# TencentARC/TVTS

Hardware: AMD Instinct MI355X
Metric: video-text pairs/sec/node, TVTSv2 pretrain step (higher is better)
Workload: dtype bf16; 1 GPU; TVTSv2 ViT-B/16 8-frame 224^2, mask 0.5, 32-token captions x4, full pretrain step (fwd+losses+bwd+HF-AdamW); pairs_per_gpu=192, global_batch=192, parallelism=dp1, hip_graph=False

## Files before the change

tvts_amd/csrc/attention.hip:

```cpp
#include "common.h"
#include <stdlib.h>

enum { MODE_FULL = 0, MODE_SPACE = 1, MODE_TIME = 2, MODE_CLS = 3 };
#ifndef TVTS_DH
#define TVTS_DH 64
#endif
#define DH TVTS_DH
#if TVTS_DH == 64
#define NS_DH dh64
#define ABI(name) tvts_attn_##name
#define VSTRIDE 160
#else
#define NS_DH dh80
#define ABI(name) tvts_attn80_##name
#define VSTRIDE 192
#endif
namespace NS_DH {
constexpr int DT = DH / 16;
constexpr int KS = (DH + 31) / 32;
constexpr int NCH = DH / 8;

struct AttnGeom {
    int B, heads, S, T, n;
    int causal;
// ... 1636 lines not shown
template <int MT, bool TR, int RS_ = 0>
__global__ __launch_bounds__(256) void attn_fwd_time_fused_kernel(AttnGeom g, const bf16* __restrict__ qkv,
                                                                  bf16* __restrict__ out, int ldo, float* __restrict__ lse2,
                                                                  float* __restrict__ cls_part) {
    extern __shared__ __attribute__((aligned(16))) char smem[];
    constexpr int RA = MT * 16, RS = RS_ ? RS_ : RA, TB = RS * VSTRIDE, NU = (MT + 1) / 2;
    constexpr int WB = TB + (DH + 2 + 2) * 4 + 1024;
    constexpr int PT = (RS * NCH + 63) / 64;
    const int lane = threadIdx.x & 63, wave = threadIdx.x >> 6;
    char* Vs = smem + wave * WB;
    char* opatch = Vs + TB + (DH + 4) * 4;
    const int chunks = (g.n + TIME_CHUNK - 1) / TIME_CHUNK;
    Grp r;
    r.h = blockIdx.x % g.heads;
    const int c = (blockIdx.x / g.heads) % chunks;
    r.b = blockIdx.x / (g.heads * chunks); r.nq = g.T; r.nk = g.T + 1;
    const int p_end = (c + 1) * TIME_CHUNK < g.n ? (c + 1) * TIME_CHUNK : g.n;
    const int gq = lane >> 4, li = lane & 15;
    const int hcol = r.h * DH;
    const int m = g.T + 1;
    float Mr = -1e30f, Lr = 0.f;
    f32x4 Or[DT];
#pragma unroll
    for (int dt = 0; dt < DT; ++dt) Or[dt] = (f32x4){0, 0, 0, 0};
    Q8Out q8o;
    q8o.init(g);

    bf16x8 qf[MT][KS], kf[MT][KS], vst[PT];
    auto issue = [&](int p) {
        r.sub = p;
#pragma unroll
        for (int t = 0; t < MT; ++t) {
            const int j = t * 16 + li;
            const bf16* rowp = qkv + (size_t)k_row<MODE_TIME>(g, r, j < m ? j : m - 1) * g.ld + hcol;
            ld_frags(rowp, gq, qf[t]);
            ld_frags(rowp + g.W, gq, kf[t]);
        }
#pragma unroll
        for (int i = 0; i < PT; ++i) {
            const int cc = lane + 64 * i, row = cc / NCH, ch = cc % NCH;
            vst[i] = row < m ? ldg8(qkv + (size_t)k_row<MODE_TIME>(g, r, row) * g.ld + 2 * g.W + hcol + ch * 8) : zero8();
        }
    };
    int p = c * TIME_CHUNK + wave;
    if (p < p_end) issue(p);
    for (; p < p_end; p += 4) {
#pragma unroll
        for (int i = 0; i < PT; ++i) {
            const int cc = lane + 64 * i, row = cc / NCH, ch = cc % NCH;
            if (row < RS) *(bf16x8*)(Vs + row * VSTRIDE + ch * 16) = vst[i];
        }
        bf16x8 qc[MT][KS], kc[MT][KS];
#pragma unroll
        for (int t = 0; t < MT; ++t)
#pragma unroll
            for (int ks = 0; ks < KS; ++ks) { qc[t][ks] = qf[t][ks]; kc[t][ks] = kf[t][ks]; }
        const bool first = p == 0;
        if (p + 4 < p_end) issue(p + 4);
        r.sub = p;
#pragma unroll
        for (int qt = 0; qt < MT; ++qt) {
            const int qj = qt * 16 + li;
            f32x4 st[2 * NU];
            float mx = -INFINITY;
#pragma unroll
            for (int t = 0; t < 2 * NU; ++t) {
                st[t] = (f32x4){-INFINITY, -INFINITY, -INFINITY, -INFINITY};
                if (t < MT) {
                    f32x4 sc = {0, 0, 0, 0};
#pragma unroll
                    for (int ks = 0; ks < KS; ++ks) sc = __builtin_amdgcn_mfma_f32_16x16x32_bf16(kc[t][ks], qc[qt][ks], sc, 0, 0, 0);
#pragma unroll
                    for (int e = 0; e < 4; ++e) {
                        const int key = t * 16 + gq * 4 + e;
                        const bool ok = key < m && !(key == 0 && qj == 0 && !first);
                        const float v = ok ? sc[e] * g.scale2 : -INFINITY;
                        st[t][e] = v;
                        mx = fmaxf(mx, v);
                    }
                }
            }
            mx = group_max(mx);
            float rs = 0.f;
#pragma unroll
            for (int t = 0; t < 2 * NU; ++t)
#pragma unroll
                for (int e = 0; e < 4; ++e) {
                    const float pp = __builtin_amdgcn_exp2f(st[t][e] - mx);
                    st[t][e] = pp;
                    rs += pp;
                }
            const float l = group_sum(rs);
            f32x4 o[DT];
#pragma unroll
            for (int dt = 0; dt < DT; ++dt) o[dt] = (f32x4){0, 0, 0, 0};
#pragma unroll
            for (int u = 0; u < NU; ++u) {
                bf16x8 pf;
#pragma unroll
                for (int j = 0; j < 8; ++j) pf[j] = (bf16)st[2 * u + (j >> 2)][j & 3];
#pragma unroll
                for (int dt = 0; dt < DT; ++dt)
                    o[dt] = __builtin_amdgcn_mfma_f32_16x16x32_bf16(frag_T_lim<TR>(Vs, u, dt, lane, RA, RS), pf, o[dt], 0, 0, 0);
            }
            {
                const float inv = 1.0f / l;
                f32x4 on[DT];
#pragma unroll
                for (int dt = 0; dt < DT; ++dt) on[dt] = o[dt] * inv;
                store_tile_rows(opatch, on, lane, [&](int rr) -> bf16* {
                    const int j = qt * 16 + rr;
                    return (j >= 1 && j < m) ? out + (size_t)k_row<MODE_TIME>(g, r, j) * ldo + hcol : nullptr; }, &q8o);
            }
            if (qj >= 1 && qj < m && gq == 0) lse2[(size_t)k_row<MODE_TIME>(g, r, qj) * g.heads + r.h] = mx + log2f(l);
            if (qt == 0) {
                const float Mn = fmaxf(Mr, mx);
                const float a = __builtin_amdgcn_exp2f(Mr - Mn), b = __builtin_amdgcn_exp2f(mx - Mn);
                Lr = Lr * a + l * b;
#pragma unroll
                for (int dt = 0; dt < DT; ++dt) Or[dt] = Or[dt] * a + o[dt] * b;
                Mr = Mn;
            }
        }
    }
    q8o.finish(g, lane);
    float* cst = (float*)(smem + wave * WB + TB);
    if (li == 0) {
        if (gq == 0) { cst[0] = Mr; cst[1] = Lr; }
#pragma unroll
        for (int dt = 0; dt < DT; ++dt)
#pragma unroll
            for (int e = 0; e < 4; ++e) cst[2 + dt * 16 + gq * 4 + e] = Or[dt][e];
    }
    __syncthreads();
    if (threadIdx.x < DH) {
        const int d = threadIdx.x;
        float M = -1e30f;
#pragma unroll
        for (int w = 0; w < 4; ++w) M = fmaxf(M, *(const float*)(smem + w * WB + TB));
        float L = 0.f, O = 0.f;
#pragma unroll
        for (int w = 0; w < 4; ++w) {
            const float* cw = (const float*)(smem + w * WB + TB);
            const float sc = __builtin_amdgcn_exp2f(cw[0] - M);
            L += cw[1] * sc;
            O += cw[2 + d] * sc;
        }
        float* cp = cls_part + ((size_t)(r.b * g.heads + r.h) * chunks + c) * (DH + 2);
        if (d == 0) { cp[0] = M; cp[1] = L; }
        cp[2 + d] = O;
    }
}

template <int MT, bool TR>
__global__ __launch_bounds__(256) void attn_fwd_seq_fused_kernel(AttnGeom g, const bf16* __restrict__ qkv,
                                                                 bf16* __restrict__ out, int ldo, float* __restrict__ lse2) {
    extern __shared__ __attribute__((aligned(16))) char smem[];
    constexpr int RA = MT * 16, TB = RA * VSTRIDE, NU = (MT + 1) / 2;
    constexpr int WB = TB + 1024;
    constexpr int PT = (RA * NCH + 63) / 64;
    const int lane = threadIdx.x & 63, wave = threadIdx.x >> 6;
    char* Vs = smem + wave * WB;
    char* opatch = Vs + TB;
    const int gq = lane >> 4, li = lane & 15;
    const int m = g.S, groups = g.B * g.heads, stride = gridDim.x * 4;
    const bool causal = g.causal != 0;

    bf16x8 qf[MT][KS], kf[MT][KS], vst[PT];
    auto issue = [&](int gid) {
        const bf16* base = qkv + (size_t)(gid / g.heads) * g.S * g.ld + (gid % g.heads) * DH;
#pragma unroll
        for (int t = 0; t < MT; ++t) {
            const int j = t * 16 + li;
            const bf16* rowp = base + (size_t)(j < m ? j : m - 1) * g.ld;
            ld_frags(rowp, gq, qf[t]);
            ld_frags(rowp + g.W, gq, kf[t]);
        }
#pragma unroll
        for (int i = 0; i < PT; ++i) {
            const int cc = lane + 64 * i, row = cc / NCH, ch = cc % NCH;
            vst[i] = row < m ? ldg8(base + (size_t)row * g.ld + 2 * g.W + ch * 8) : zero8();
        }
    };
    int gid = blockIdx.x * 4 + wave;
    if (gid < groups) issue(gid);
    for (; gid < groups; gid += stride) {
#pragma unroll
        for (int i = 0; i < PT; ++i) {
            const int cc = lane + 64 * i, row = cc / NCH, ch = cc % NCH;
            if (row < RA) *(bf16x8*)(Vs + row * VSTRIDE + ch * 16) = vst[i];
        }
        bf16x8 qc[MT][KS], kc[MT][KS];
#pragma unroll
        for (int t = 0; t < MT; ++t)
#pragma unroll
            for (int ks = 0; ks < KS; ++ks) { qc[t][ks] = qf[t][ks]; kc[t][ks] = kf[t][ks]; }
        if (gid + stride < groups) issue(gid + stride);
        const int h = gid % g.heads;
        const size_t row0 = (size_t)(gid / g.heads) * g.S;
        const int hcol = h * DH;
#pragma unroll
        for (int qt = 0; qt < MT; ++qt) {
            const int qj = qt * 16 + li;
            f32x4 st[2 * NU];
            float mx = -INFINITY;
#pragma unroll
            for (int t = 0; t < 2 * NU; ++t) {
                st[t] = (f32x4){-INFINITY, -INFINITY, -INFINITY, -INFINITY};
                if (t < MT) {
                    f32x4 sc = {0, 0, 0, 0};
#pragma unroll
                    for (int ks = 0; ks < KS; ++ks) sc = __builtin_amdgcn_mfma_f32_16x16x32_bf16(kc[t][ks], qc[qt][ks], sc, 0, 0, 0);
#pragma unroll
                    for (int e = 0; e < 4; ++e) {
                        const int key = t * 16 + gq * 4 + e;
                        const bool ok = key < m && !(causal && key > qj);
                        const float v = ok ? sc[e] * g.scale2 : -INFINITY;
                        st[t][e] = v;
                        mx = fmaxf(mx, v);
                    }
                }
            }
            mx = group_max(mx);
            float rs = 0.f;
#pragma unroll
            for (int t = 0; t < 2 * NU; ++t)
#pragma unroll
                for (int e = 0; e < 4; ++e) {
                    const float pp = __builtin_amdgcn_exp2f(st[t][e] - mx);
                    st[t][e] = pp;
                    rs += pp;
                }
            const float l = group_sum(rs);
            f32x4 o[DT];
#pragma unroll
            for (int dt = 0; dt < DT; ++dt) o[dt] = (f32x4){0, 0, 0, 0};
#pragma unroll
            for (int u = 0; u < NU; ++u) {
                bf16x8 pf;
#pragma unroll
                for (int j = 0; j < 8; ++j) pf[j] = (bf16)st[2 * u + (j >> 2)][j & 3];
#pragma unroll
                for (int dt = 0; dt < DT; ++dt)
                    o[dt] = __builtin_amdgcn_mfma_f32_16x16x32_bf16(frag_T_lim<TR>(Vs, u, dt, lane, RA), pf, o[dt], 0, 0, 0);
            }
            {
                const float inv = 1.0f / l;
                f32x4 on[DT];
#pragma unroll
                for (int dt = 0; dt < DT; ++dt) on[dt] = o[dt] * inv;
                store_tile_rows(opatch, on, lane, [&](int rr) -> bf16* {
                    const int j = qt * 16 + rr;
                    return j < m ? out + (row0 + j) * ldo + hcol : nullptr; });
            }
            if (qj < m && gq == 0) lse2[(row0 + qj) * g.heads + h] = mx + log2f(l);
        }
    }
}

#define SEQ_BWD_WAVES 2
template <int MT, bool TR>
__global__ __launch_bounds__(64 * SEQ_BWD_WAVES) void attn_bwd_seq_fused_kernel(AttnGeom g, const bf16* __restrict__ qkv,
                                                                               const bf16* __restrict__ dO, int lddo,
                                                                               const float* __restrict__ lse2,
                                                                               bf16* __restrict__ dqkv, int lddq) {
    extern __shared__ __attribute__((aligned(16))) char smem[];
    constexpr int RA = MT * 16, TB = RA * VSTRIDE, NU = (MT + 1) / 2;
    constexpr int WB = 4 * TB + 2 * RA * 4 + 1024;
    constexpr int PT = (RA * NCH + 63) / 64;
    const int lane = threadIdx.x & 63, wave = threadIdx.x >> 6;
    char* base = smem + wave * WB;
    char* Qs = base;
    char* Ks = Qs + TB;
    char* Vs = Ks + TB;
    char* Ds = Vs + TB;
    float* st_lse = (float*)(Ds + TB);
    float* st_dl = st_lse + RA;
    char* opatch = (char*)(st_dl + RA);
    const int gq = lane >> 4, li = lane & 15;
    const int m = g.S, groups = g.B * g.heads, stride = gridDim.x * SEQ_BWD_WAVES;
    const bool causal = g.causal != 0;

    bf16x8 stg[4][PT];
    float lse_pf = 0.f;
    auto issue = [&](int gid) {
        const int h = gid % g.heads;
        const size_t row0 = (size_t)(gid / g.heads) * g.S;
#pragma unroll
        for (int t = 0; t < 4; ++t) {
            const bf16* src = t == 3 ? dO + h * DH : qkv + t * g.W + h * DH;
            const int ld = t == 3 ? lddo : g.ld;
#pragma unroll
            for (int i = 0; i < PT; ++i) {
                const int cc = lane + 64 * i, row = cc / NCH, ch = cc % NCH;
                stg[t][i] = row < m ? ldg8(src + (row0 + row) * ld + ch * 8) : zero8();
            }
        }
        if (lane < m) lse_pf = lse2[(row0 + lane) * g.heads + h];
    };
    int gid = blockIdx.x * SEQ_BWD_WAVES + wave;
    if (gid < groups) issue(gid);
    for (; gid < groups; gid += stride) {
#pragma unroll
        for (int t = 0; t < 4; ++t)
#pragma unroll
            for (int i = 0; i < PT; ++i) {
// ... 417 lines not shown
}

static __global__ __launch_bounds__(256) void attn_delta_tail_kernel(const bf16* __restrict__ dO, int lddo, const bf16* __restrict__ O,
                                                              int ldo, int B, int S, int nq, const int* __restrict__ qpos, int heads,
                                                              float* __restrict__ delta) {
    const long rh = (long)blockIdx.x * 256 + threadIdx.x;
    if (rh >= (long)B * nq * heads) return;
    const int h = (int)(rh % heads), qi = (int)((rh / heads) % nq), b = (int)(rh / ((long)heads * nq));
    const size_t row = (size_t)b * S + (qpos ? qpos[b] : S - nq) + qi;
    float s = 0.f;
#pragma unroll
    for (int ch = 0; ch < NCH; ++ch) {
        const bf16x8 a = ldg8(dO + row * lddo + h * DH + ch * 8);
        const bf16x8 c = ldg8(O + row * ldo + h * DH + ch * 8);
#pragma unroll
        for (int e = 0; e < 8; ++e) s += (float)a[e] * (float)c[e];
    }
    delta[row * heads + h] = s;
}
extern "C" int ABI(fwd_tail)(const void* qkv, int ld, int B, int heads, int S, int nq, void* out, int ldo, float* lse2,
                             hipStream_t stream) {
    ATTN_OPTS(0);
    AttnGeom g;
    int rc = make_geom(g, MODE_CLS, B, heads, S, 0, 0, 0, ld);
    if (rc) return rc;
    if (nq < 1 || nq > 16 || nq > S || ldo % 4) return TVTS_EINVAL;
    g.cls_nq = nq; g.cls_q0 = S - nq;
    DISPATCH_MODE(attn_fwd_kernel, MODE_CLS, dim3(B * heads), dim3(256), 0, stream, g, (const bf16*)qkv, (bf16*)out, ldo, lse2);
    TVTS_LAUNCH_CHECK();
    return TVTS_OK;
}
extern "C" int ABI(bwd_tail)(const void* qkv, int ld, int B, int heads, int S, int nq, const void* dO, int lddo, const void* O,
                             int ldo, const float* lse2, float* delta, void* dqkv, int lddq, hipStream_t stream) {
    ATTN_OPTS(0);
    AttnGeom g;
    int rc = make_geom(g, MODE_CLS, B, heads, S, 0, 0, 0, ld);
    if (rc) return rc;
    if (nq < 1 || nq > 16 || nq > S || lddo % 8 || ldo % 8 || lddq % 4) return TVTS_EINVAL;
    g.cls_nq = nq; g.cls_q0 = S - nq;
    const long total = (long)B * nq * heads;
    hipLaunchKernelGGL(attn_delta_tail_kernel, dim3((unsigned)((total + 255) / 256)), dim3(256), 0, stream, (const bf16*)dO, lddo,
                       (const bf16*)O, ldo, B, S, nq, (const int*)nullptr, heads, delta);
    DISPATCH_MODE(attn_bwd_dq_kernel, MODE_CLS, dim3(B * heads), dim3(256), 0, stream, g, (const bf16*)qkv, (const bf16*)dO, lddo,
                  lse2, delta, (bf16*)dqkv, lddq);
    const int blocks = ceil_div(B * heads * ceil_div(S, 16), 4);
    DISPATCH_MODE(attn_bwd_dkv_kernel, MODE_CLS, dim3(blocks), dim3(256), 0, stream, g, (const bf16*)qkv, (const bf16*)dO, lddo,
                  lse2, delta, (bf16*)dqkv, lddq, (float*)nullptr);
    TVTS_LAUNCH_CHECK();
    return TVTS_OK;
}

extern "C" int ABI(fwd_rowq)(const void* qkv, int ld, int B, int heads, int S, const int* qpos, void* out, int ldo, float* lse2,
                             hipStream_t stream) {
    ATTN_OPTS(0);
    AttnGeom g;
    int rc = make_geom(g, MODE_CLS, B, heads, S, 0, 0, 0, ld);
    if (rc) return rc;
    if (!qpos || ldo % 4) return TVTS_EINVAL;
    g.cls_qpos = qpos;
    DISPATCH_MODE(attn_fwd_kernel, MODE_CLS, dim3(B * heads), dim3(256), 0, stream, g, (const bf16*)qkv, (bf16*)out, ldo, lse2);
    TVTS_LAUNCH_CHECK();
    return TVTS_OK;
}
extern "C" int ABI(bwd_rowq)(const void* qkv, int ld, int B, int heads, int S, const int* qpos, const void* dO, int lddo,
                             const void* O, int ldo, const float* lse2, float* delta, void* dqkv, int lddq, hipStream_t stream) {
    ATTN_OPTS(0);
    AttnGeom g;
    int rc = make_geom(g, MODE_CLS, B, heads, S, 0, 0, 0, ld);
    if (rc) return rc;
    if (!qpos || lddo % 8 || ldo % 8 || lddq % 4) return TVTS_EINVAL;
    g.cls_qpos = qpos;
    const long total = (long)B * heads;
    hipLaunchKernelGGL(attn_delta_tail_kernel, dim3((unsigned)((total + 255) / 256)), dim3(256), 0, stream, (const bf16*)dO, lddo,
                       (const bf16*)O, ldo, B, S, 1, qpos, heads, delta);
    DISPATCH_MODE(attn_bwd_dq_kernel, MODE_CLS, dim3(B * heads), dim3(256), 0, stream, g, (const bf16*)qkv, (const bf16*)dO, lddo,
                  lse2, delta, (bf16*)dqkv, lddq);
    const int blocks = ceil_div(B * heads * ceil_div(S, 16), 4);
    DISPATCH_MODE(attn_bwd_dkv_kernel, MODE_CLS, dim3(blocks), dim3(256), 0, stream, g, (const bf16*)qkv, (const bf16*)dO, lddo,
                  lse2, delta, (bf16*)dqkv, lddq, (float*)nullptr);
    TVTS_LAUNCH_CHECK();
    return TVTS_OK;
}

extern "C" int ABI(cls_finalize)(const float* cls_acc, int B, int heads, int S, void* dqkv, int lddq,
                                      hipStream_t stream) {
    const int total = B * heads * 3 * DH;
    hipLaunchKernelGGL(attn_cls_finalize_kernel, dim3(ceil_div(total, 256)), dim3(256), 0, stream, cls_acc, B, heads, S,
                       heads * DH, 0, (bf16*)dqkv, lddq, 1);
    TVTS_LAUNCH_CHECK();
    return TVTS_OK;
}

static __global__ void zero_f32_kernel(float* __restrict__ p, int n) {
    const int i = blockIdx.x * 256 + threadIdx.x;
    if (i < n) p[i] = 0.f;
}

static int bwd_impl(int mode, const void* qkv, int ld, int B, int heads, int S, int T, int n, int causal,
                    const void* dO, int lddo, const void* O, int ldo, const float* lse2, float* delta, void* dqkv,
                    int lddq, float* cls_acc, long cls_acc_elems, void* q8out, int ldq8, const float* q8_scale, float* q8_amax,
                    int opts, hipStream_t stream) {
    if (mode == MODE_CLS) return TVTS_EINVAL;
    ATTN_OPTS(opts);
    AttnGeom g;
    int rc = make_geom(g, mode, B, heads, S, T, n, causal, ld);
    if (rc) return rc;
    if (lddo % 8 || ldo % 8 || lddq % 4) return TVTS_EINVAL;
    if (q8out) {
        if (ldq8 != lddq || lddq % 8 || !q8_scale) return TVTS_EINVAL;
        g.q8_ref = (const bf16*)dqkv; g.q8 = (unsigned char*)q8out; g.q8_scale = q8_scale; g.q8_amax = q8_amax;
    }
    const bool divided = mode == MODE_SPACE || mode == MODE_TIME;
    if (fused && use_tr && mode == MODE_FULL && S <= 32) {
        const int MT = ceil_div(S, 16), groups = B * heads;
        const int lds_bytes = SEQ_BWD_WAVES * (4 * MT * 16 * VSTRIDE + 2 * MT * 16 * 4 + 1024);
        const int want = ceil_div(groups, SEQ_BWD_WAVES);
        const int blocks = want < 768 ? want : 768;
        if (MT == 1) hipLaunchKernelGGL((attn_bwd_seq_fused_kernel<1, true>), dim3(blocks), dim3(64 * SEQ_BWD_WAVES), lds_bytes, stream, g, (const bf16*)qkv, (const bf16*)dO, lddo, lse2, (bf16*)dqkv, lddq);
        else hipLaunchKernelGGL((attn_bwd_seq_fused_kernel<2, true>), dim3(blocks), dim3(64 * SEQ_BWD_WAVES), lds_bytes, stream, g, (const bf16*)qkv, (const bf16*)dO, lddo, lse2, (bf16*)dqkv, lddq);
        TVTS_LAUNCH_CHECK();
        return TVTS_OK;
    }
    const bool fused_space = fused && use_tr && mode == MODE_SPACE && n + 1 <= FUSED_MAX_TILES * 16;
    const bool fused_time = fused && use_tr && mode == MODE_TIME && T + 1 <= 32;
    const int want_parts = fused_space ? T : fused_time ? ceil_div(n, TIME_CHUNK) : 0;
    const bool parts_ok = want_parts > 0 && cls_acc && cls_acc_elems >= (long)B * heads * want_parts * 3 * DH;
    g.cls_parts = parts_ok ? want_parts : 0;
    g.ablate = (opts >> 4) & 7;
    g.q8_only = (q8out && (opts & 128)) ? 1 : 0;
    if (divided && !parts_ok) {
        if (!cls_acc || cls_acc_elems < (long)B * heads * 3 * DH) return TVTS_EINVAL;
        const int nz = B * heads * 3 * DH;
        hipLaunchKernelGGL(zero_f32_kernel, dim3(ceil_div(nz, 256)), dim3(256), 0, stream, cls_acc, nz);
    }
    typedef void (*FusedKern)(AttnGeom, const bf16*, const bf16*, int, const float*, const float*, bf16*, int, float*);
    if (fused_space || fused_time) {
        hipLaunchKernelGGL(attn_delta_kernel, dim3((unsigned)(((long)B * heads + 255) / 256)), dim3(256), 0, stream,
                           (const bf16*)dO, lddo, (const bf16*)O, ldo, B, S, heads, delta);
        FusedKern kern = nullptr;
        int lds_bytes = 0, blocks = 0, threads = 0, slot = 0;
        if (fused_space) {
            const int MT = (n + 1 + 15) / 16, RA = MT * 16;
            lds_bytes = 4 * RA * VSTRIDE + 2 * RA * (int)sizeof(float) + (FUSED_THREADS / 64) * 1024;
            switch (MT) {
                case 1: kern = attn_bwd_space_fused_kernel<1, true>; break;
                case 2: kern = attn_bwd_space_fused_kernel<2, true>; break;
                case 3: kern = attn_bwd_space_fused_kernel<3, true>; break;
                case 4: kern = attn_bwd_space_fused_kernel<4, true>; break;
                case 5: kern = attn_bwd_space_fused_kernel<5, true>; break;
                case 6: kern = attn_bwd_space_fused_kernel<6, true>; break;
                default: kern = attn_bwd_space_fused_kernel<7, true>; break;
            }
            blocks = B * heads * T; threads = FUSED_THREADS; slot = MT;
        } else {
            const int MT = (T + 1 + 15) / 16, RA = MT * 16;
            const int RS = (MT == 2 && T + 1 <= 20) ? 20 : RA;
            lds_bytes = 4 * (4 * RS * VSTRIDE + 2 * RA * 4 + 3 * DH * 4 + 1024);
            kern = MT == 1 ? attn_bwd_time_fused_kernel<1, true> : RS == 20 ? attn_bwd_time_fused_kernel<2, true, 20> : attn_bwd_time_fused_kernel<2, true>;
            blocks = B * heads * ceil_div(n, TIME_CHUNK); threads = 256; slot = FUSED_MAX_TILES + MT;
        }
        (void)slot;
        if (hipFuncSetAttribute((const void*)kern, hipFuncAttributeMaxDynamicSharedMemorySize, lds_bytes) != hipSuccess)
            return TVTS_EINVAL;
        hipLaunchKernelGGL(kern, dim3(blocks), dim3(threads), lds_bytes, stream, g, (const bf16*)qkv, (const bf16*)dO, lddo,
                           lse2, delta, (bf16*)dqkv, lddq, cls_acc);
        TVTS_LAUNCH_CHECK();
        const int total = B * heads * 3 * DH;
        hipLaunchKernelGGL(attn_cls_finalize_kernel, dim3(ceil_div(total, 256)), dim3(256), 0, stream, cls_acc, B, heads, S,
                           heads * DH, 1, (bf16*)dqkv, lddq, g.cls_parts ? g.cls_parts : 1, g.q8, g.q8_scale, g.q8_amax);
        TVTS_LAUNCH_CHECK();
        return TVTS_OK;
    }
    if (q8out) return TVTS_EINVAL;
    rc = ABI(delta)(dO, lddo, O, ldo, B * S, heads, delta, stream);
    if (rc) return rc;
    rc = ABI(bwd_dq)(mode, qkv, ld, B, heads, S, T, n, causal, dO, lddo, lse2, delta, dqkv, lddq, opts, stream);
    if (rc) return rc;
    rc = ABI(bwd_dkv)(mode, qkv, ld, B, heads, S, T, n, causal, dO, lddo, lse2, delta, dqkv, lddq, cls_acc, opts, stream);
    if (rc) return rc;
    if (divided) {
        rc = ABI(bwd_dq)(MODE_CLS, qkv, ld, B, heads, S, T, n, 0, dO, lddo, lse2, delta, dqkv, lddq, opts, stream);
        if (rc) return rc;
        rc = ABI(cls_finalize)(cls_acc, B, heads, S, dqkv, lddq, stream);
    }
    return rc;
}
extern "C" int ABI(bwd)(int mode, const void* qkv, int ld, int B, int heads, int S, int T, int n, int causal,
                        const void* dO, int lddo, const void* O, int ldo, const float* lse2, float* delta, void* dqkv,
                        int lddq, float* cls_acc, long cls_acc_elems, int opts, hipStream_t stream) {
    return bwd_impl(mode, qkv, ld, B, heads, S, T, n, causal, dO, lddo, O, ldo, lse2, delta, dqkv, lddq, cls_acc, cls_acc_elems,
                    nullptr, 0, nullptr, nullptr, opts, stream);
}
extern "C" int ABI(bwd_q8)(int mode, const void* qkv, int ld, int B, int heads, int S, int T, int n, int causal,
                           const void* dO, int lddo, const void* O, int ldo, const float* lse2, float* delta, void* dqkv,
                           int lddq, float* cls_acc, long cls_acc_elems, void* q8out, int ldq8, const float* q8_scale,
                           float* q8_amax, int opts, hipStream_t stream) {
    if (!q8out) return TVTS_EINVAL;
    return bwd_impl(mode, qkv, ld, B, heads, S, T, n, causal, dO, lddo, O, ldo, lse2, delta, dqkv, lddq, cls_acc, cls_acc_elems,
                    q8out, ldq8, q8_scale, q8_amax, opts, stream);
}

static int fwd_divided_impl(int mode, const void* qkv, int ld, int B, int heads, int S, int T, int n, void* out, int ldo,
                            float* lse2, float* cls_ws, long cls_ws_elems, void* q8out, int ldq8, const float* q8_scale,
                            float* q8_amax, int opts, hipStream_t stream) {
    if (mode != MODE_SPACE && mode != MODE_TIME) return TVTS_EINVAL;
    ATTN_OPTS(opts);
    AttnGeom g;
    int rc = make_geom(g, mode, B, heads, S, T, n, 0, ld);
    if (rc) return rc;
    if (ldo % 4) return TVTS_EINVAL;
    if (q8out) {
        if (ldq8 != ldo || ldo % 8 || !q8_scale) return TVTS_EINVAL;
        g.q8_ref = (const bf16*)out; g.q8 = (unsigned char*)q8out; g.q8_scale = q8_scale; g.q8_amax = q8_amax;
        g.q8_only = (opts & 128) ? 1 : 0;
    }
    const bool fs = fused && use_tr && mode == MODE_SPACE && n + 1 <= FUSED_MAX_TILES * 16;
    const bool ft = fused && use_tr && mode == MODE_TIME && T + 1 <= 32;
    const int G = mode == MODE_SPACE ? T : ceil_div(n, TIME_CHUNK);
    if ((fs || ft) && cls_ws && cls_ws_elems >= (long)B * heads * G * (DH + 2)) {
        typedef void (*Kern)(AttnGeom, const bf16*, bf16*, int, float*, float*);
        Kern kern = nullptr;
        int lds_bytes, blocks;
        if (fs) {
            const int MT = (n + 1 + 15) / 16;
            switch (MT) {
                case 1: kern = attn_fwd_space_fused_kernel<1, true>; break;
                case 2: kern = attn_fwd_space_fused_kernel<2, true>; break;
                case 3: kern = attn_fwd_space_fused_kernel<3, true>; break;
                case 4: kern = attn_fwd_space_fused_kernel<4, true>; break;
                case 5: kern = attn_fwd_space_fused_kernel<5, true>; break;
                case 6: kern = attn_fwd_space_fused_kernel<6, true>; break;
                default: kern = attn_fwd_space_fused_kernel<7, true>; break;
            }
            lds_bytes = 2 * MT * 16 * VSTRIDE + 4 * 1024;
            blocks = B * heads * T;
        } else {
            const int MT = (T + 1 + 15) / 16;
            const int RS = (MT == 2 && T + 1 <= 20) ? 20 : MT * 16;
            kern = MT == 1 ? attn_fwd_time_fused_kernel<1, true> : RS == 20 ? attn_fwd_time_fused_kernel<2, true, 20> : attn_fwd_time_fused_kernel<2, true>;
            lds_bytes = 4 * (RS * VSTRIDE + (DH + 4) * 4 + 1024);
            blocks = B * heads * G;
        }
        hipLaunchKernelGGL(kern, dim3(blocks), dim3(256), lds_bytes, stream, g, (const bf16*)qkv, (bf16*)out, ldo, lse2, cls_ws);
        TVTS_LAUNCH_CHECK();
        hipLaunchKernelGGL(attn_cls_merge_kernel, dim3(B * heads), dim3(DH <= 64 ? 64 : 128), 0, stream, cls_ws, G, heads, S,
                           (bf16*)out, ldo, lse2, g.q8, g.q8_scale, g.q8_amax);
        TVTS_LAUNCH_CHECK();
        return TVTS_OK;
    }
    if (q8out) return TVTS_EINVAL;
    rc = ABI(fwd)(mode, qkv, ld, B, heads, S, T, n, 0, out, ldo, lse2, opts, stream);
    if (rc) return rc;
    return ABI(fwd)(MODE_CLS, qkv, ld, B, heads, S, T, n, 0, out, ldo, lse2, opts, stream);
}
extern "C" int ABI(fwd_divided)(int mode, const void* qkv, int ld, int B, int heads, int S, int T, int n, void* out, int ldo,
                                float* lse2, float* cls_ws, long cls_ws_elems, int opts, hipStream_t stream) {
    return fwd_divided_impl(mode, qkv, ld, B, heads, S, T, n, out, ldo, lse2, cls_ws, cls_ws_elems, nullptr, 0, nullptr, nullptr, opts, stream);
}
extern "C" int ABI(fwd_divided_q8)(int mode, const void* qkv, int ld, int B, int heads, int S, int T, int n, void* out, int ldo,
                                   float* lse2, float* cls_ws, long cls_ws_elems, void* q8out, int ldq8, const float* q8_scale,
                                   float* q8_amax, int opts, hipStream_t stream) {
    if (!q8out) return TVTS_EINVAL;
    return fwd_divided_impl(mode, qkv, ld, B, heads, S, T, n, out, ldo, lse2, cls_ws, cls_ws_elems, q8out, ldq8, q8_scale, q8_amax, opts, stream);
}
```

Before: 1420 pairs/s.

## Pack multiple spatial positions per MFMA tile in divided time attention

```diff
diff --git a/tvts_amd/csrc/attention.hip b/tvts_amd/csrc/attention.hip
--- a/tvts_amd/csrc/attention.hip
+++ b/tvts_amd/csrc/attention.hip
@@ -1812,6 +1812,418 @@
     }
 }
 
+__device__ __forceinline__ bf16x8 frag_T_pk(const char* tile, const char* crow, int dt, int lane) {
+    const int gq = lane >> 4, i = lane & 15;
+    const s16x4 t0 = __builtin_amdgcn_ds_read_tr16_b64_v4i16((LDS_PTR(s16x4))(tile + (gq * 4 + (i >> 2)) * VSTRIDE + dt * 32 + (i & 3) * 8));
+    const s16x4 t1 = __builtin_amdgcn_ds_read_tr16_b64_v4i16((LDS_PTR(s16x4))(crow + (i >> 2) * VSTRIDE + dt * 32 + (i & 3) * 8));
+    const bf16x4 b0 = __builtin_bit_cast(bf16x4, t0), b1 = __builtin_bit_cast(bf16x4, t1);
+    bf16x8 out;
+#pragma unroll
+    for (int e = 0; e < 4; ++e) out[e] = b0[e];
+    out[4] = gq == 0 ? b1[0] : (bf16)0.f;
+    out[5] = out[6] = out[7] = (bf16)0.f;
+    return out;
+}
+
+struct PkRow {
+    int fr, sl;
+    __device__ __forceinline__ void init(int r, int T, int n) { fr = (r % T) * n; sl = r / T; }
+    __device__ __forceinline__ int row(int p0, int ns) const { return fr + p0 + (sl < ns ? sl : ns - 1); }
+};
+__device__ __forceinline__ unsigned pk_block_diag(int li, int gq, int T) {
+    const int P = 16 / T;
+    unsigned bd = 0;
+#pragma unroll
+    for (int e = 0; e < 4; ++e) {
+        const int kr = gq * 4 + e;
+        if (kr < P * T && li < P * T && kr / T == li / T) bd |= 1u << e;
+    }
+    return bd;
+}
+
+template <bool TR>
+__global__ __launch_bounds__(256, DH == 64 ? 4 : 3) void attn_fwd_time_packed_kernel(AttnGeom g, const bf16* __restrict__ qkv,
+                                                                      bf16* __restrict__ out, int ldo, float* __restrict__ lse2,
+                                                                      float* __restrict__ cls_part) {
+    static_assert(TR, "packed TIME kernels: ds_read_tr only");
+    extern __shared__ __attribute__((aligned(16))) char smem[];
+    constexpr int TB = 16 * VSTRIDE, WB = TB + (DH + 4) * 4 + 1024, PTV = (16 * NCH + 63) / 64;
+    const int lane = threadIdx.x & 63, wave = threadIdx.x >> 6;
+    const int gq = lane >> 4, li = lane & 15;
+    char* Vc = smem;
+    char* Vs = smem + 4 * VSTRIDE + wave * WB;
+    float* cst = (float*)(Vs + TB);
+    char* opatch = Vs + TB + (DH + 4) * 4;
+    const int T = g.T, n = g.n, P = 16 / T;
+    const int chunks = (n + TIME_CHUNK - 1) / TIME_CHUNK;
+    const int h = blockIdx.x % g.heads, c = (blockIdx.x / g.heads) % chunks, b = blockIdx.x / (g.heads * chunks);
+    const int s0 = c * TIME_CHUNK, s_end = s0 + TIME_CHUNK < n ? s0 + TIME_CHUNK : n;
+    const int ntiles = (s_end - s0 + P - 1) / P;
+    const int hcol = h * DH;
+    const bf16* cls = qkv + (size_t)(b * g.S) * g.ld + hcol;
+    const bf16* prow = cls + (size_t)g.ld;
+    for (int i = threadIdx.x; i < 4 * NCH; i += 256)
+        *(bf16x8*)(Vc + (i / NCH) * VSTRIDE + (i % NCH) * 16) = i < NCH ? ldg8(cls + 2 * g.W + (i % NCH) * 8) : zero8();
+    bf16x8 qcf[KS], kcf[KS];
+    ld_frags(cls, gq, qcf);
+    ld_frags(cls + g.W, gq, kcf);
+    PkRow rq, rst, rv[PTV];
+    rq.init(li, T, n);
+    rst.init(lane >> 2, T, n);
+#pragma unroll
+    for (int i = 0; i < PTV; ++i) rv[i].init(((lane + 64 * i) / NCH) & 15, T, n);
+    const unsigned bd = pk_block_diag(li, gq, T);
+    Q8Out q8o;
+    q8o.init(g);
+
+    float Mr = -1e30f, Lr = 0.f;
+    f32x4 Or[DT];
+#pragma unroll
+    for (int dt = 0; dt < DT; ++dt) Or[dt] = (f32x4){0, 0, 0, 0};
+    if (c == 0 && wave == 0) {
+        f32x4 s = {0, 0, 0, 0};
+#pragma unroll
+        for (int ks = 0; ks < KS; ++ks) s = __builtin_amdgcn_mfma_f32_16x16x32_bf16(kcf[ks], qcf[ks], s, 0, 0, 0);
+        Mr = s[0] * g.scale2;
+        Lr = 1.f;
+#pragma unroll
+        for (int dt = 0; dt < DT; ++dt)
+#pragma unroll
+            for (int e = 0; e < 4; ++e) Or[dt][e] = (float)cls[2 * g.W + dt * 16 + gq * 4 + e];
+    }
+    __syncthreads();
+
+    bf16x8 qf[KS], kf[KS], vst[PTV];
+    auto issue = [&](int tl) {
+        const int p0 = s0 + tl * P, ns = s_end - p0 < P ? s_end - p0 : P;
+        const bf16* rowp = prow + (size_t)rq.row(p0, ns) * g.ld;
+        ld_frags(rowp, gq, qf);
+        ld_frags(rowp + g.W, gq, kf);
+#pragma unroll
+        for (int i = 0; i < PTV; ++i) {
+            const int cc = lane + 64 * i;
+            vst[i] = cc < 16 * NCH ? ldg8(prow + (size_t)rv[i].row(p0, ns) * g.ld + 2 * g.W + (cc % NCH) * 8) : zero8();
+        }
+    };
+    int tl = wave;
+    if (tl < ntiles) issue(tl);
+    for (; tl < ntiles; tl += 4) {
+#pragma unroll
+        for (int i = 0; i < PTV; ++i) {
+            const int cc = lane + 64 * i;
+            if (cc < 16 * NCH) *(bf16x8*)(Vs + (cc / NCH) * VSTRIDE + (cc % NCH) * 16) = vst[i];
+        }
+        asm volatile("" ::: "memory");
+        bf16x8 qc[KS], kc[KS];
+#pragma unroll
+        for (int ks = 0; ks < KS; ++ks) { qc[ks] = qf[ks]; kc[ks] = kf[ks]; }
+        const int p0 = s0 + tl * P, ns = s_end - p0 < P ? s_end - p0 : P, nr = ns * T;
+        if (tl + 4 < ntiles) issue(tl + 4);
+
+        f32x4 sc = {0, 0, 0, 0}, scl = {0, 0, 0, 0}, sq = {0, 0, 0, 0};
+#pragma unroll
+        for (int ks = 0; ks < KS; ++ks) {
+            sc = __builtin_amdgcn_mfma_f32_16x16x32_bf16(kc[ks], qc[ks], sc, 0, 0, 0);
+            scl = __builtin_amdgcn_mfma_f32_16x16x32_bf16(kcf[ks], qc[ks], scl, 0, 0, 0);
+            sq = __builtin_amdgcn_mfma_f32_16x16x32_bf16(kc[ks], qcf[ks], sq, 0, 0, 0);
+        }
+        const float sC = scl[0] * g.scale2;
+        float st[4], mx = -INFINITY;
+#pragma unroll
+        for (int e = 0; e < 4; ++e) {
+            st[e] = (bd >> e) & 1 ? sc[e] * g.scale2 : -INFINITY;
+            mx = fmaxf(mx, st[e]);
+        }
+        mx = fmaxf(group_max(mx), sC);
+        float rs = 0.f;
+#pragma unroll
+        for (int e = 0; e < 4; ++e) { st[e] = __builtin_amdgcn_exp2f(st[e] - mx); rs += st[e]; }
+        const float pC = __builtin_amdgcn_exp2f(sC - mx);
+        const float l = group_sum(rs) + pC;
+        bf16x8 pf;
+#pragma unroll
+        for (int e = 0; e < 4; ++e) pf[e] = (bf16)st[e];
+        pf[4] = gq == 0 ? (bf16)pC : (bf16)0.f;
+        pf[5] = pf[6] = pf[7] = (bf16)0.f;
+        float s2[4], m2 = -INFINITY;
+#pragma unroll
+        for (int e = 0; e < 4; ++e) {
+            s2[e] = gq * 4 + e < nr ? sq[e] * g.scale2 : -INFINITY;
+            m2 = fmaxf(m2, s2[e]);
+        }
+        const float Mn = fmaxf(Mr, group_max(m2));
+        const float a = __builtin_amdgcn_exp2f(Mr - Mn);
+        float r2 = 0.f;
+        bf16x8 pq;
+#pragma unroll
+        for (int e = 0; e < 4; ++e) {
+            const float pp = __builtin_amdgcn_exp2f(s2[e] - Mn);
+            r2 += pp;
+            pq[e] = (bf16)pp;
+        }
+        pq[4] = pq[5] = pq[6] = pq[7] = (bf16)0.f;
+        Lr = Lr * a + group_sum(r2);
+        Mr = Mn;
+        f32x4 o[DT];
+#pragma unroll
+        for (int dt = 0; dt < DT; ++dt) {
+            const bf16x8 vt = frag_T_pk(Vs, Vc, dt, lane);
+            o[dt] = __builtin_amdgcn_mfma_f32_16x16x32_bf16(vt, pf, (f32x4){0, 0, 0, 0}, 0, 0, 0);
+            Or[dt] = __builtin_amdgcn_mfma_f32_16x16x32_bf16(vt, pq, Or[dt] * a, 0, 0, 0);
+        }
+        {
+            const float inv = 1.0f / l;
+            f32x4 on[DT];
+#pragma unroll
+            for (int dt = 0; dt < DT; ++dt) on[dt] = o[dt] * inv;
+            store_tile_rows(opatch, on, lane, [&](int) -> bf16* {
+                return rst.sl < ns ? out + (size_t)(b * g.S + 1 + rst.row(p0, ns)) * ldo + hcol : nullptr; }, &q8o);
+        }
+        if (gq == 0 && rq.sl < ns) lse2[(size_t)(b * g.S + 1 + rq.row(p0, ns)) * g.heads + h] = mx + log2f(l);
+        asm volatile("" ::: "memory");
+    }
+    q8o.finish(g, lane);
+    if (li == 0) {
+        if (gq == 0) { cst[0] = Mr; cst[1] = Lr; }
+#pragma unroll
+        for (int dt = 0; dt < DT; ++dt) *(f32x4*)(cst + 2 + dt * 16 + gq * 4) = Or[dt];
+    }
+    __syncthreads();
+    if (threadIdx.x < DH) {
+        const int d = threadIdx.x;
+        const char* w0 = smem + 4 * VSTRIDE + TB;
+        float M = -1e30f;
+#pragma unroll
+        for (int w = 0; w < 4; ++w) M = fmaxf(M, *(const float*)(w0 + w * WB));
+        float L = 0.f, O = 0.f;
+#pragma unroll
+        for (int w = 0; w < 4; ++w) {
+            const float* cw = (const float*)(w0 + w * WB);
+            const float sc = __builtin_amdgcn_exp2f(cw[0] - M);
+            L += cw[1] * sc;
+            O += cw[2 + d] * sc;
+        }
+        float* cp = cls_part + ((size_t)(b * g.heads + h) * chunks + c) * (DH + 2);
+        if (d == 0) { cp[0] = M; cp[1] = L; }
+        cp[2 + d] = O;
+    }
+}
+
+template <bool TR>
+__global__ __launch_bounds__(256, DH == 64 ? 3 : 2) void attn_bwd_time_packed_kernel(AttnGeom g, const bf16* __restrict__ qkv,
+                                                                      const bf16* __restrict__ dO, int lddo,
+                                                                      const float* __restrict__ lse2, const float* __restrict__ delta,
+                                                                      bf16* __restrict__ dqkv, int lddq, float* __restrict__ cls_acc) {
+    static_assert(TR, "packed TIME kernels: ds_read_tr only");
+    extern __shared__ __attribute__((aligned(16))) char smem[];
+    constexpr int TB = 16 * VSTRIDE, CB = 4 * VSTRIDE, WB = 4 * TB + 6 * 16 * 4 + 3 * DH * 4 + 1024, PTV = (16 * NCH + 63) / 64;
+    const int lane = threadIdx.x & 63, wave = threadIdx.x >> 6;
+    const int gq = lane >> 4, li = lane & 15;
+    const char* Qc = smem;
+    const char* Kc = smem + CB;
+    const char* Vc = smem + 2 * CB;
+    const char* Dc = smem + 3 * CB;
+    char* base = smem + 4 * CB + wave * WB;
+    char* Qs = base;
+    char* Ks = Qs + TB;
+    char* Vs = Ks + TB;
+    char* Ds = Vs + TB;
+    float* st_lse = (float*)(Ds + TB);
+    float* st_dl = st_lse + 16;
+    float* st_pc = st_dl + 16;
+    float* st_dsc = st_pc + 16;
+    float* st_pq = st_dsc + 16;
+    float* st_dsq = st_pq + 16;
+    float* csum = st_dsq + 16;
+    char* opatch = (char*)(csum + 3 * DH);
+    const int T = g.T, n = g.n, P = 16 / T;
+    const int chunks = (n + TIME_CHUNK - 1) / TIME_CHUNK;
+    const int h = blockIdx.x % g.heads, c = (blockIdx.x / g.heads) % chunks, b = blockIdx.x / (g.heads * chunks);
+    const int s0 = c * TIME_CHUNK, s_end = s0 + TIME_CHUNK < n ? s0 + TIME_CHUNK : n;
+    const int ntiles = (s_end - s0 + P - 1) / P;
+    const int hcol = h * DH;
+    const size_t ocls = (size_t)(b * g.S) * g.heads + h;
+    const float lse_c = lse2[ocls], dl_c = delta[ocls];
+    for (int i = lane; i < 3 * DH; i += 64) csum[i] = 0.f;
+    for (int i = threadIdx.x; i < 4 * 4 * NCH; i += 256) {
+        const int t = i / (4 * NCH), row = (i / NCH) % 4, ch = i % NCH;
+        const bf16* src = t == 3 ? dO + (size_t)(b * g.S) * lddo + hcol : qkv + (size_t)(b * g.S) * g.ld + t * g.W + hcol;
+        *(bf16x8*)(smem + t * CB + row * VSTRIDE + ch * 16) = row == 0 ? ldg8(src + ch * 8) : zero8();
+    }
+    PkRow rq, rst, rv[PTV];
+    rq.init(li, T, n);
+    rst.init(lane >> 2, T, n);
+#pragma unroll
+    for (int i = 0; i < PTV; ++i) rv[i].init(((lane + 64 * i) / NCH) & 15, T, n);
+    const unsigned bd = pk_block_diag(li, gq, T);
+    const size_t rb = (size_t)(b * g.S + 1);
+    Q8Out q8o;
+    q8o.init(g);
+    __syncthreads();
+
+    float pcc = 0.f, dscc = 0.f;
+    if (c == 0 && wave == 0) {
+        f32x4 s = {0, 0, 0, 0}, dp = {0, 0, 0, 0};
+#pragma unroll
+        for (int ks = 0; ks < KS; ++ks) {
+            s = __builtin_amdgcn_mfma_f32_16x16x32_bf16(frag_row(Kc, 0, ks, gq), frag_row(Qc, 0, ks, gq), s, 0, 0, 0);
+            dp = __builtin_amdgcn_mfma_f32_16x16x32_bf16(frag_row(Vc, 0, ks, gq), frag_row(Dc, 0, ks, gq), dp, 0, 0, 0);
+        }
+        pcc = __builtin_amdgcn_exp2f(s[0] * g.scale2 - lse_c);
+        dscc = pcc * (dp[0] - dl_c) * g.scale;
+    }
+
+    bf16x8 stg[4][PTV];
+    float lse_pf = 0.f;
+    auto issue = [&](int tl) {
+        const int p0 = s0 + tl * P, ns = s_end - p0 < P ? s_end - p0 : P;
+        const bool ld = !(g.ablate & 4);
+#pragma unroll
+        for (int t = 0; t < 4; ++t) {
+            const bf16* src = t == 3 ? dO + rb * lddo + hcol : qkv + rb * g.ld + t * g.W + hcol;
+            const int ldt = t == 3 ? lddo : g.ld;
+#pragma unroll
+            for (int i = 0; i < PTV; ++i) {
+                const int cc = lane + 64 * i;
+                stg[t][i] = cc < 16 * NCH && ld ? ldg8(src + (size_t)rv[i].row(p0, ns) * ldt + (cc % NCH) * 8) : zero8();
+            }
+        }
+        if (lane < 16) lse_pf = lse2[(rb + rq.row(p0, ns)) * g.heads + h];
+    };
+    int tl = wave;
+    if (tl < ntiles) issue(tl);
+    for (; tl < ntiles; tl += 4) {
+#pragma unroll
+        for (int t = 0; t < 4; ++t)
+#pragma unroll
+            for (int i = 0; i < PTV; ++i) {
+                const int cc = lane + 64 * i;
+                if (cc < 16 * NCH) *(bf16x8*)(base + t * TB + (cc / NCH) * VSTRIDE + (cc % NCH) * 16) = stg[t][i];
+            }
+        if (lane < 16) st_lse[lane] = lse_pf;
+        asm volatile("" ::: "memory");
+        const int p0 = s0 + tl * P, ns = s_end - p0 < P ? s_end - p0 : P, nr = ns * T;
+        if (tl + 4 < ntiles) issue(tl + 4);
+        const bool qok = rq.sl < ns;
+
+        if (!(g.ablate & 1)) {
+            bf16x8 qf[KS], dof[KS], kf[KS], vf[KS];
+#pragma unroll
+            for (int ks = 0; ks < KS; ++ks) {
+                qf[ks] = frag_row(Qs, li, ks, gq); dof[ks] = frag_row(Ds, li, ks, gq);
+                kf[ks] = frag_row(Ks, li, ks, gq); vf[ks] = frag_row(Vs, li, ks, gq);
+            }
+            f32x4 sc = {0, 0, 0, 0}, dp = {0, 0, 0, 0}, scl = {0, 0, 0, 0}, dpl = {0, 0, 0, 0}, sq = {0, 0, 0, 0}, dpq = {0, 0, 0, 0};
+#pragma unroll
+            for (int ks = 0; ks < KS; ++ks) {
+                const bf16x8 kcb = frag_row(Kc, 0, ks, gq), vcb = frag_row(Vc, 0, ks, gq);
+                const bf16x8 qcb = frag_row(Qc, 0, ks, gq), dcb = frag_row(Dc, 0, ks, gq);
+                sc = __builtin_amdgcn_mfma_f32_16x16x32_bf16(kf[ks], qf[ks], sc, 0, 0, 0);
+                dp = __builtin_amdgcn_mfma_f32_16x16x32_bf16(vf[ks], dof[ks], dp, 0, 0, 0);
+                scl = __builtin_amdgcn_mfma_f32_16x16x32_bf16(kcb, qf[ks], scl, 0, 0, 0);
+                dpl = __builtin_amdgcn_mfma_f32_16x16x32_bf16(vcb, dof[ks], dpl, 0, 0, 0);
+                sq = __builtin_amdgcn_mfma_f32_16x16x32_bf16(kf[ks], qcb, sq, 0, 0, 0);
+                dpq = __builtin_amdgcn_mfma_f32_16x16x32_bf16(vf[ks], dcb, dpq, 0, 0, 0);
+            }
+            const float lse = st_lse[li];
+            float pp[4], part = 0.f;
+#pragma unroll
+            for (int e = 0; e < 4; ++e) {
+                pp[e] = (bd >> e) & 1 ? __builtin_amdgcn_exp2f(sc[e] * g.scale2 - lse) : 0.f;
+                part += pp[e] * dp[e];
+            }
+            const float pc = qok ? __builtin_amdgcn_exp2f(scl[0] * g.scale2 - lse) : 0.f;
+            const float dlt = group_sum(part) + pc * dpl[0];
+            const float dsc = pc * (dpl[0] - dlt) * g.scale;
+            bf16x8 dsf, dsq;
+            float pqv[4], dsqv[4];
+#pragma unroll
+            for (int e = 0; e < 4; ++e) {
+                dsf[e] = (bf16)(pp[e] * (dp[e] - dlt) * g.scale);
+                pqv[e] = gq * 4 + e < nr ? __builtin_amdgcn_exp2f(sq[e] * g.scale2 - lse_c) : 0.f;
+                dsqv[e] = pqv[e] * (dpq[e] - dl_c) * g.scale;
+                dsq[e] = (bf16)dsqv[e];
+            }
+            dsf[4] = gq == 0 ? (bf16)dsc : (bf16)0.f;
+            dsq[4] = gq == 0 ? (bf16)dscc : (bf16)0.f;
+            dsf[5] = dsf[6] = dsf[7] = dsq[5] = dsq[6] = dsq[7] = (bf16)0.f;
+            f32x4 acc[DT], accq[DT];
+#pragma unroll
+            for (int dt = 0; dt < DT; ++dt) {
+                const bf16x8 kt = frag_T_pk(Ks, Kc, dt, lane);
+                acc[dt] = __builtin_amdgcn_mfma_f32_16x16x32_bf16(kt, dsf, (f32x4){0, 0, 0, 0}, 0, 0, 0);
+                accq[dt] = __builtin_amdgcn_mfma_f32_16x16x32_bf16(kt, dsq, (f32x4){0, 0, 0, 0}, 0, 0, 0);
+            }
+            store_tile_rows(opatch, acc, lane, [&](int) -> bf16* {
+                return rst.sl < ns ? dqkv + (rb + rst.row(p0, ns)) * lddq + hcol : nullptr; }, &q8o);
+            if (li == 0) {
+#pragma unroll
+                for (int dt = 0; dt < DT; ++dt) *(f32x4*)(csum + 2 * DH + dt * 16 + gq * 4) += accq[dt];
+#pragma unroll
+                for (int e = 0; e < 4; ++e) { st_pq[gq * 4 + e] = pqv[e]; st_dsq[gq * 4 + e] = dsqv[e]; }
+            }
+            if (gq == 0) { st_dl[li] = dlt; st_pc[li] = pc; st_dsc[li] = dsc; }
+        }
+
+        asm volatile("" ::: "memory");
+        if (!(g.ablate & 2)) {
+            f32x4 sc = {0, 0, 0, 0}, dp = {0, 0, 0, 0};
+#pragma unroll
+            for (int ks = 0; ks < KS; ++ks) {
+                sc = __builtin_amdgcn_mfma_f32_16x16x32_bf16(frag_row(Qs, li, ks, gq), frag_row(Ks, li, ks, gq), sc, 0, 0, 0);
+                dp = __builtin_amdgcn_mfma_f32_16x16x32_bf16(frag_row(Ds, li, ks, gq), frag_row(Vs, li, ks, gq), dp, 0, 0, 0);
+            }
+            const f32x4 l4 = *(const f32x4*)(st_lse + gq * 4), d4 = *(const f32x4*)(st_dl + gq * 4);
+            const f32x4 pc4 = *(const f32x4*)(st_pc + gq * 4), ds4 = *(const f32x4*)(st_dsc + gq * 4);
+            bf16x8 pf, dsf, pcf, dscf;
+#pragma unroll
+            for (int e = 0; e < 4; ++e) {
+                const float pp = (bd >> e) & 1 ? __builtin_amdgcn_exp2f(sc[e] * g.scale2 - l4[e]) : 0.f;
+                pf[e] = (bf16)pp;
+                dsf[e] = (bf16)(pp * (dp[e] - d4[e]) * g.scale);
+                pcf[e] = (bf16)pc4[e];
+                dscf[e] = (bf16)ds4[e];
+            }
+            pf[4] = gq == 0 ? (bf16)st_pq[li] : (bf16)0.f;
+            dsf[4] = gq == 0 ? (bf16)st_dsq[li] : (bf16)0.f;
+            pcf[4] = gq == 0 ? (bf16)pcc : (bf16)0.f;
+            dscf[4] = gq == 0 ? (bf16)dscc : (bf16)0.f;
+            pf[5] = pf[6] = pf[7] = dsf[5] = dsf[6] = dsf[7] = (bf16)0.f;
+            pcf[5] = pcf[6] = pcf[7] = dscf[5] = dscf[6] = dscf[7] = (bf16)0.f;
+            f32x4 dv[DT], dk[DT];
+#pragma unroll
+            for (int dt = 0; dt < DT; ++dt) {
+                const bf16x8 dtf = frag_T_pk(Ds, Dc, dt, lane), qtf = frag_T_pk(Qs, Qc, dt, lane);
+                dv[dt] = __builtin_amdgcn_mfma_f32_16x16x32_bf16(dtf, pf, (f32x4){0, 0, 0, 0}, 0, 0, 0);
+                dk[dt] = __builtin_amdgcn_mfma_f32_16x16x32_bf16(qtf, dsf, (f32x4){0, 0, 0, 0}, 0, 0, 0);
+                const f32x4 vc = __builtin_amdgcn_mfma_f32_16x16x32_bf16(dtf, pcf, (f32x4){0, 0, 0, 0}, 0, 0, 0);
+                const f32x4 kc = __builtin_amdgcn_mfma_f32_16x16x32_bf16(qtf, dscf, (f32x4){0, 0, 0, 0}, 0, 0, 0);
+                if (li == 0) {
+                    *(f32x4*)(csum + dt * 16 + gq * 4) += kc;
+                    *(f32x4*)(csum + DH + dt * 16 + gq * 4) += vc;
+                }
+            }
+            auto krowp = [&](int third) {
+                return [&, third](int) -> bf16* {
+                    return rst.sl < ns ? dqkv + (rb + rst.row(p0, ns)) * lddq + third * g.W + hcol : nullptr; };
+            };
+            store_tile_rows(opatch, dk, lane, krowp(1), &q8o);
+            store_tile_rows(opatch, dv, lane, krowp(2), &q8o);
+        }
+        pcc = dscc = 0.f;
+        asm volatile("" ::: "memory");
+    }
+    q8o.finish(g, lane);
+    __syncthreads();
+    if (threadIdx.x < 3 * DH) {
+        const int i = threadIdx.x;
+        const char* w0 = smem + 4 * CB + 4 * TB + 6 * 16 * 4 + i * 4;
+        const float v = *(const float*)(w0) + *(const float*)(w0 + WB) + *(const float*)(w0 + 2 * WB) + *(const float*)(w0 + 3 * WB);
+        if (g.cls_parts) cls_acc[(((size_t)(b * g.heads + h) * g.cls_parts + c) * 3) * DH + i] = v;
+        else atomicAdd(cls_acc + ((size_t)(b * g.heads + h) * 3) * DH + i, v);
+    }
+}
+
 template <int MT, bool TR>
 __global__ __launch_bounds__(256) void attn_fwd_seq_fused_kernel(AttnGeom g, const bf16* __restrict__ qkv,
                                                                  bf16* __restrict__ out, int ldo, float* __restrict__ lse2) {
@@ -2535,6 +2947,10 @@
                 default: kern = attn_bwd_space_fused_kernel<7, true>; break;
             }
             blocks = B * heads * T; threads = FUSED_THREADS; slot = MT;
+        } else if (T <= 16) {
+            lds_bytes = 4 * 4 * VSTRIDE + 4 * (4 * 16 * VSTRIDE + 6 * 16 * 4 + 3 * DH * 4 + 1024);
+            kern = attn_bwd_time_packed_kernel<true>;
+            blocks = B * heads * ceil_div(n, TIME_CHUNK); threads = 256;
         } else {
             const int MT = (T + 1 + 15) / 16, RA = MT * 16;
             const int RS = (MT == 2 && T + 1 <= 20) ? 20 : RA;
@@ -2617,6 +3033,10 @@
             }
             lds_bytes = 2 * MT * 16 * VSTRIDE + 4 * 1024;
             blocks = B * heads * T;
+        } else if (T <= 16) {
+            kern = attn_fwd_time_packed_kernel<true>;
+            lds_bytes = 4 * VSTRIDE + 4 * (16 * VSTRIDE + (DH + 4) * 4 + 1024);
+            blocks = B * heads * G;
         } else {
             const int MT = (T + 1 + 15) / 16;
             const int RS = (MT == 2 && T + 1 <= 20) ? 20 : MT * 16;
```

Result: no change. 1423 pairs/s (median of 6 runs) (+0.2%).
